# HanielUlises/GCN-GrabCut

Hardware: AMD Instinct MI355X
Metric: images/sec end-to-end mask (DUTS-shape batch) (higher is better)
Workload: dtype f32

## Files before the change

### gcn-grabcut_amd/csrc/ggc_ccl.h

```cpp
#pragma once
#include <hip/hip_runtime.h>
#include <cstdint>

namespace ggc {

__device__ __forceinline__ int ccl_find(const int32_t* parent, int i) {
    int p = __hip_atomic_load(&parent[i], __ATOMIC_RELAXED, __HIP_MEMORY_SCOPE_AGENT);
    while (p != i) { i = p; p = __hip_atomic_load(&parent[i], __ATOMIC_RELAXED, __HIP_MEMORY_SCOPE_AGENT); }
    return i;
}
__device__ __forceinline__ void ccl_union(int32_t* parent, int a, int b) {
    for (;;) {
        a = ccl_find(parent, a); b = ccl_find(parent, b);
        if (a == b) return;
        if (a < b) { const int t = a; a = b; b = t; }
        const int old = atomicMin(&parent[a], b);
        if (old == a) return;
        a = old;
    }
}

__host__ __device__ inline int ccl_run_start_lane(unsigned long long starts, int lane) {
    const unsigned long long below = starts & ((2ull << lane) - 1ull);
#if defined(__HIP_DEVICE_COMPILE__)
    return 63 - __clzll((long long)below);
#else
    return 63 - __builtin_clzll(below);
#endif
}
__host__ __device__ inline int ccl_run_length(unsigned long long starts, unsigned long long vmask, int lane) {
    const unsigned long long stop = (starts | ~vmask) >> lane >> 1;
#if defined(__HIP_DEVICE_COMPILE__)
    return stop ? __ffsll((long long)stop) : 64 - lane;
#else
    return stop ? __builtin_ffsll((long long)stop) : 64 - lane;
#endif
}

__device__ __forceinline__ int ccl_run_first(bool on, bool same_left, int p) {
    const int lane = threadIdx.x & 63;
    const unsigned long long starts = __ballot(on && (!same_left || lane == 0));
    return p - (lane - ccl_run_start_lane(starts, lane));
}

template <int CONN, class Joined>
__device__ __forceinline__ void ccl_merge_pixel(int32_t* par, int p, int x, bool has_up, int W, size_t flat, Joined joined) {
    static_assert(CONN == 4 || CONN == 8, "4 or 8 neighbours");
    const bool left = x > 0 && joined(p - 1);
    if (left && (flat & 63) == 0) ccl_union(par, p, p - 1);
    if (!has_up) return;
    if constexpr (CONN == 4) {
        if (joined(p - W) && !(left && joined(p - W - 1))) ccl_union(par, p, p - W);
    } else {
        const bool up = joined(p - W);
        const bool ul = x > 0 && joined(p - W - 1), ur = x + 1 < W && joined(p - W + 1);
        if (left) {
            if (ur && !up) ccl_union(par, p, p - W + 1);
        } else if (up) {
            ccl_union(par, p, p - W);
        } else {
            if (ul) ccl_union(par, p, p - W - 1);
            if (ur) ccl_union(par, p, p - W + 1);
        }
    }
}

__device__ __forceinline__ int ccl_compress(int32_t* par, int p) { const int r = ccl_find(par, p); par[p] = r; return r; }
__device__ __forceinline__ void ccl_count_runs(bool valid, bool same_left, unsigned long long vmask, int32_t* counts, size_t cell) {
    const int lane = threadIdx.x & 63;
    const unsigned long long starts = __ballot(valid && (!same_left || lane == 0));
    if (valid && ((starts >> lane) & 1ull)) atomicAdd(&counts[cell], ccl_run_length(starts, vmask, lane));
}

__host__ __device__ inline unsigned long long ccl_best_key(int area, int root) {
    return ((unsigned long long)(unsigned)area << 32) | (unsigned long long)(0xFFFFFFFFu - (unsigned)root);
}
__host__ __device__ inline int ccl_best_root(unsigned long long key) { return (int)(0xFFFFFFFFu - (unsigned)(key & 0xFFFFFFFFull)); }

}
```

### gcn-grabcut_amd/csrc/ggc_slic.hip

```cpp
#include "ggc_internal.h"
#include "ggc_ccl.h"
#include "ggc_math.h"
#include <cmath>
#include <vector>

namespace ggc {

__global__ void k_minmax_init(int B, uint32_t* mm) {
    const int i = blockIdx.x * blockDim.x + threadIdx.x;
    if (i < B) { mm[2 * i] = 0xFFFFFFFFu; mm[2 * i + 1] = 0u; }
}

__global__ void __launch_bounds__(256) k_minmax(size_t n, const float* __restrict__ img, uint32_t* mm) {
    const float* im = img + (size_t)blockIdx.y * n;
    float lo = INFINITY, hi = -INFINITY;
    for (size_t i = (size_t)blockIdx.x * blockDim.x + threadIdx.x; i < n; i += (size_t)gridDim.x * blockDim.x) {
        const float v = im[i];
        lo = fminf(lo, v); hi = fmaxf(hi, v);
    }
    for (int o = 32; o > 0; o >>= 1) { lo = fminf(lo, __shfl_xor(lo, o, 64)); hi = fmaxf(hi, __shfl_xor(hi, o, 64)); }
    __shared__ float s_lo[4], s_hi[4];
    if ((threadIdx.x & 63) == 0) { s_lo[threadIdx.x >> 6] = lo; s_hi[threadIdx.x >> 6] = hi; }
    __syncthreads();
    if (threadIdx.x == 0) {
// ... 83 lines not shown
__global__ void __launch_bounds__(256) k_gauss_v(int H, int W, const float* __restrict__ in, GaussW g, float* __restrict__ out) {
    const int col = blockIdx.x * 256 + threadIdx.x;
    if (col >= 3 * W) return;
    const size_t n = (size_t)H * W * 3;
    const float* im = in + (size_t)blockIdx.z * n + col;
    float* o = out + (size_t)blockIdx.z * n + col;
    const int y0 = blockIdx.y * GV_ROWS;
    double v[2 * R + 1];
#pragma unroll
    for (int j = 0; j < 2 * R; ++j) v[j + 1] = (double)im[(size_t)reflect_sym(y0 - R + j, H) * W * 3];
#pragma unroll 4
    for (int y = y0; y < min(y0 + GV_ROWS, H); ++y) {
#pragma unroll
        for (int j = 0; j < 2 * R; ++j) v[j] = v[j + 1];
        v[2 * R] = (double)im[(size_t)reflect_sym(y + R, H) * W * 3];
        double tmp = v[R] * g.w[R];
#pragma unroll
        for (int k = 0; k < R; ++k) tmp += (v[k] + v[2 * R - k]) * g.w[k];
        o[(size_t)y * W * 3] = (float)tmp;
    }
}

__global__ void __launch_bounds__(256) k_scale(size_t n, const float* __restrict__ in, float scale,
                                               float* __restrict__ out) {
    const size_t i = (size_t)blockIdx.x * blockDim.x + threadIdx.x;
    if (i < n) out[i] = in[i] * scale;
}

struct SlicGeom {
    int H, W, K;
    int ny, nx, start_y, start_x, step_y, step_x;
    int win_y, win_x;
    float sw;
};

__device__ __forceinline__ int4 slic_window(float cy, float cx, const SlicGeom& g) {
    if (cy != cy || cx != cx) return make_int4(0, 0, 0, 0);
    float fy0 = cy - (float)(2 * g.win_y); if (!(fy0 > 0.0f)) fy0 = 0.0f;
    float fy1 = cy + (float)(2 * g.win_y) + 1.0f; if (!(fy1 < (float)g.H)) fy1 = (float)g.H;
    float fx0 = cx - (float)(2 * g.win_x); if (!(fx0 > 0.0f)) fx0 = 0.0f;
    float fx1 = cx + (float)(2 * g.win_x) + 1.0f; if (!(fx1 < (float)g.W)) fx1 = (float)g.W;
    return make_int4((int)fy0, (int)fy1, (int)fx0, (int)fx1);
}

__global__ void k_init_centers(SlicGeom g, float* __restrict__ centers, int4* __restrict__ bounds) {
    const int k = blockIdx.x * blockDim.x + threadIdx.x;
    if (k >= g.K) return;
    const size_t o = (size_t)blockIdx.y * g.K + k;
    const float cy = (float)(g.start_y + (k / g.nx) * g.step_y);
    const float cx = (float)(g.start_x + (k % g.nx) * g.step_x);
    centers[o * 5 + 0] = cy; centers[o * 5 + 1] = cx;
    centers[o * 5 + 2] = 0.0f; centers[o * 5 + 3] = 0.0f; centers[o * 5 + 4] = 0.0f;
    bounds[o] = slic_window(cy, cx, g);
}

struct Cand { int k, y0, y1, x0, x1; float cy, cx, c0, c1, c2; };

constexpr int TILE_W = 32, TILE_H = 16;

typedef float v2f __attribute__((ext_vector_type(2)));

__global__ void __launch_bounds__(256) k_slic_assign(SlicGeom g, const float* __restrict__ image,
                                                     const float* __restrict__ centers,
                                                     const int4* __restrict__ bounds,
                                                     int32_t* __restrict__ labels, int32_t* __restrict__ stale) {
    __shared__ Cand cand[256];
    __shared__ int wcount[4];
    const int tid = threadIdx.x, lane = tid & 63, wave = tid >> 6;
    const int b = blockIdx.z;
    const int tx0 = blockIdx.x * TILE_W, ty0 = blockIdx.y * TILE_H;
    const int px = tx0 + (wave & 1) * 16 + (lane & 15), pya = ty0 + (wave >> 1) * 8 + (lane >> 4), pyb = pya + 4;
    const bool ina = px < g.W && pya < g.H, inb = px < g.W && pyb < g.H;
    const size_t P = (size_t)g.H * g.W;
    const size_t pa = (size_t)b * P + (size_t)pya * g.W + px, pb = pa + (size_t)4 * g.W;
    v2f i0 = 0.f, i1 = 0.f, i2 = 0.f;
    if (ina) { i0.x = image[3 * pa]; i1.x = image[3 * pa + 1]; i2.x = image[3 * pa + 2]; }
    if (inb) { i0.y = image[3 * pb]; i1.y = image[3 * pb + 1]; i2.y = image[3 * pb + 2]; }
    const v2f fy = {(float)pya, (float)pyb};
    const float fx = (float)px;
    float best_a = INFINITY, best_b = INFINITY;
    int lab_a = -1, lab_b = -1;
    const float* cen = centers + (size_t)b * g.K * 5;
    const int4* bnd = bounds + (size_t)b * g.K;
    for (int base = 0; base < g.K; base += 256) {
        const int k = base + tid;
        bool hit = false;
        int4 bd = make_int4(0, 0, 0, 0);
        if (k < g.K) {
            bd = bnd[k];
            hit = bd.x < ty0 + TILE_H && bd.y > ty0 && bd.z < tx0 + TILE_W && bd.w > tx0 && bd.y > bd.x && bd.w > bd.z;
        }
        const unsigned long long bal = __ballot(hit);
        const int pre = __popcll(bal & ((1ull << lane) - 1ull));
        if (lane == 0) wcount[wave] = __popcll(bal);
        __syncthreads();
        int off = 0, total = 0;
#pragma unroll
        for (int w = 0; w < 4; ++w) { if (w < wave) off += wcount[w]; total += wcount[w]; }
        if (hit) {
            Cand c;
            c.k = k; c.y0 = bd.x; c.y1 = bd.y; c.x0 = bd.z; c.x1 = bd.w;
            c.cy = cen[k * 5 + 0]; c.cx = cen[k * 5 + 1];
            c.c0 = cen[k * 5 + 2]; c.c1 = cen[k * 5 + 3]; c.c2 = cen[k * 5 + 4];
            cand[off + pre] = c;
        }
        __syncthreads();
        for (int i = 0; i < total; ++i) {
            const Cand& c = cand[i];
            const bool xin = (unsigned)(px - c.x0) < (unsigned)(c.x1 - c.x0);
            const unsigned hgt = (unsigned)(c.y1 - c.y0);
            const bool hit_a = xin && (unsigned)(pya - c.y0) < hgt, hit_b = xin && (unsigned)(pyb - c.y0) < hgt;
            if (!(hit_a || hit_b)) continue;
            const v2f ty = c.cy - fy;
            const float tx = c.cx - fx;
            v2f dd = (ty * ty + tx * tx) * g.sw;
            v2f t = i0 - c.c0;
            v2f dc = t * t;
            t = i1 - c.c1; dc += t * t;
            t = i2 - c.c2; dc += t * t;
            dd += dc;
            if (hit_a && best_a > dd.x) { best_a = dd.x; lab_a = c.k; }
            if (hit_b && best_b > dd.y) { best_b = dd.y; lab_b = c.k; }
        }
        __syncthreads();
    }
    bool none = false;
    if (ina) { if (lab_a >= 0) labels[pa] = lab_a; else none = true; }
    if (inb) { if (lab_b >= 0) labels[pb] = lab_b; else none = true; }
    if (none) atomicOr(&stale[b], 1);
}

constexpr int UPD_LANES = 8, UPD_GROUPS = 64 / UPD_LANES, UPD_CH = 8;
constexpr int UPD_CAP = 32;
constexpr int UPD_FOLD_UNROLL = 4;
static_assert(UPD_CAP >= 2 * UPD_LANES && UPD_CAP % UPD_FOLD_UNROLL == 0, "a fold per chunk, or fold reads past the list");

__device__ __forceinline__ void upd_wave_sync() {
    __builtin_amdgcn_fence(__ATOMIC_ACQ_REL, "wavefront");
    __builtin_amdgcn_wave_barrier();
}

__global__ void __launch_bounds__(256) k_slic_update(SlicGeom g, const float* __restrict__ image,
                                                     const int32_t* __restrict__ labels,
                                                     const int32_t* __restrict__ stale,
                                                     float* __restrict__ centers, int4* __restrict__ bounds) {
    __shared__ float upd_buf[4][UPD_CAP][UPD_GROUPS * 3];
    const int lane = threadIdx.x & 63, sub = lane / UPD_LANES, sl = lane % UPD_LANES;
    const int k = (blockIdx.x * 4 + (threadIdx.x >> 6)) * UPD_GROUPS + sub;
    const bool live = k < g.K;
    const int b = blockIdx.y;
    const size_t o = (size_t)b * g.K + (live ? k : 0);
    int4 bd = live ? bounds[o] : make_int4(0, 0, 0, 0);
    if (live && stale[b]) bd = make_int4(0, g.H, 0, g.W);
    const size_t P = (size_t)g.H * g.W;
    const int32_t* lb = labels + (size_t)b * P;
    const float* im = image + (size_t)b * P * 3;
    float s = 0.f;
    int cnt = 0, isy = 0, isx = 0;
    int nbuf = 0;
    float* const put = &upd_buf[threadIdx.x >> 6][0][sub * 3];
    const float* const get = put + min(sl, 2);
    auto fold = [&]() {
        upd_wave_sync();
        for (int i = 0; __any(i < nbuf); i += UPD_FOLD_UNROLL) {
            float v[UPD_FOLD_UNROLL];
#pragma unroll
            for (int u = 0; u < UPD_FOLD_UNROLL; ++u) v[u] = get[(i + u) * (UPD_GROUPS * 3)];
#pragma unroll
            for (int u = 0; u < UPD_FOLD_UNROLL; ++u) s += i + u < nbuf ? v[u] : 0.f;
        }
        nbuf = 0;
        upd_wave_sync();
    };
    const int rows = bd.y - bd.x, chunks = (bd.w - bd.z + UPD_LANES - 1) / UPD_LANES;
    int rows_max = rows, chunks_max = chunks;
#pragma unroll
    for (int off = UPD_LANES; off < 64; off <<= 1) {
        rows_max = max(rows_max, __shfl_xor(rows_max, off, 64));
        chunks_max = max(chunks_max, __shfl_xor(chunks_max, off, 64));
    }
    rows_max = __builtin_amdgcn_readfirstlane(rows_max);
    chunks_max = __builtin_amdgcn_readfirstlane(chunks_max);
    const int32_t* lane_p = lb + (size_t)bd.x * g.W + bd.z + sl;
    const int nvc = (bd.w - bd.z - sl + UPD_LANES - 1) / UPD_LANES;
    auto load_row = [&](int ry, int c0, int (&lab)[UPD_CH]) {
        const int32_t* rp = lane_p + (size_t)ry * g.W + c0 * UPD_LANES;
        const int nv = ry < rows ? nvc - c0 : 0;
#pragma unroll
        for (int c = 0; c < UPD_CH; ++c) lab[c] = c < nv ? rp[c * UPD_LANES] : -1;
    };
    const int nblk = (chunks_max + UPD_CH - 1) / UPD_CH, total = rows_max * nblk;
    int cur[UPD_CH], nxt[UPD_CH];
    if (total > 0) load_row(0, 0, cur);
    asm volatile("" :: "v"(cur[0]), "v"(cur[1]), "v"(cur[2]), "v"(cur[3]), "v"(cur[4]), "v"(cur[5]), "v"(cur[6]), "v"(cur[7]));
    int ry = 0, cb = 0;
    for (int t = 0; t < total; ++t) {
        int ry_n = ry, cb_n = cb + 1;
        if (cb_n == nblk) { cb_n = 0; ++ry_n; }
        load_row(ry_n, cb_n * UPD_CH, nxt);
        bool hit[UPD_CH], some = false;
#pragma unroll
        for (int c = 0; c < UPD_CH; ++c) { hit[c] = cur[c] == k && live; some |= hit[c]; }
        if (__any(some)) {
            const int y = bd.x + ry, x0 = bd.z + cb * UPD_CH * UPD_LANES + sl;
            const float* px = im + ((size_t)y * g.W + x0) * 3;
            float v0[UPD_CH], v1[UPD_CH], v2[UPD_CH];
#pragma unroll
            for (int c = 0; c < UPD_CH; ++c) {
                const float* q = hit[c] ? px + c * UPD_LANES * 3 : im;
                v0[c] = q[0]; v1[c] = q[1]; v2[c] = q[2];
            }
#pragma unroll
            for (int c = 0; c < UPD_CH; ++c) {
                const unsigned long long bal = __ballot(hit[c]);
                if (bal) {
                    if (__any(nbuf > UPD_CAP - UPD_LANES)) fold();
                    const unsigned int m = (unsigned int)(bal >> (sub * UPD_LANES)) & ((1u << UPD_LANES) - 1u);
                    const int n = __popc(m);
                    cnt += n; isy += n * y;
                    if (hit[c]) {
                        float* e = put + (nbuf + __popc(m & ((1u << sl) - 1u))) * (UPD_GROUPS * 3);
                        e[0] = v0[c]; e[1] = v1[c]; e[2] = v2[c];
                        isx += x0 + c * UPD_LANES;
                    }
                    nbuf += n;
                }
            }
        }
#pragma unroll
        for (int c = 0; c < UPD_CH; ++c) cur[c] = nxt[c];
        ry = ry_n; cb = cb_n;
    }
    fold();
    const float s0 = __shfl(s, lane - sl, 64), s1 = __shfl(s, lane - sl + 1, 64), s2 = __shfl(s, lane - sl + 2, 64);
#pragma unroll
    for (int off = 1; off < UPD_LANES; off <<= 1) isx += __shfl_xor(isx, off, 64);
    float sy = (float)isy, sx = (float)isx;
    if (live && (isy >= (1 << 24) || isx >= (1 << 24))) {
        sy = 0.f; sx = 0.f;
        for (int y = bd.x; y < bd.y; ++y)
            for (int x = bd.z; x < bd.w; ++x)
                if (lb[(size_t)y * g.W + x] == k) { sy += (float)y; sx += (float)x; }
    }
    if (!live || sl != 0) return;
    const float n = (float)cnt;
    const float cy = sy / n, cx = sx / n;
    centers[o * 5 + 0] = cy; centers[o * 5 + 1] = cx;
    centers[o * 5 + 2] = s0 / n; centers[o * 5 + 3] = s1 / n; centers[o * 5 + 4] = s2 / n;
    bounds[o] = slic_window(cy, cx, g);
}

__global__ void __launch_bounds__(64) k_connectivity_seq(int H, int W, const int32_t* __restrict__ labels,
                                                         int min_size, int max_size,
                                                         int32_t* __restrict__ queue,
                                                         int32_t* __restrict__ out, int32_t* __restrict__ n_nodes) {
    if (threadIdx.x != 0) return;
    const int b = blockIdx.x;
    const size_t P = (size_t)H * W;
    const int32_t* lb = labels + (size_t)b * P;
    int32_t* o = out + (size_t)b * P;
    int32_t* q = queue + (size_t)b * (size_t)(max_size > 0 ? max_size : 1);
    int cur = 0;
    for (int y = 0; y < H; ++y)
        for (int x = 0; x < W; ++x) {
            const int p0 = y * W + x;
            if (o[p0] >= 0) continue;
            int adjacent = 0;
            const int label = lb[p0];
            o[p0] = cur;
            int size = 1, visited = 0;
            q[0] = p0;
            while (visited < size && size < max_size) {
                const int pc = q[visited];
                const int yc = pc / W, xc = pc - yc * W;
#pragma unroll
                for (int i = 0; i < 4; ++i) {
                    const int xx = xc + (i == 0 ? 1 : i == 1 ? -1 : 0);
                    const int yy = yc + (i == 2 ? 1 : i == 3 ? -1 : 0);
                    if (xx < 0 || xx >= W || yy < 0 || yy >= H) continue;
                    const int pp = yy * W + xx;
                    const int op = o[pp];
                    if (op == -1 && lb[pp] == label) {
                        o[pp] = cur;
                        q[size] = pp;
                        size += 1;
                        if (size >= max_size) break;
                    } else if (op >= 0 && op != cur) {
                        adjacent = op;
                    }
                }
                visited += 1;
            }
            if (size < min_size) {
                for (int i = 0; i < size; ++i) o[q[i]] = adjacent;
            } else {
                cur += 1;
            }
        }
    n_nodes[b] = cur > 0 ? cur : 1;
}

struct CnDims { int B, H, W, P, min_size, max_size; };

__global__ void __launch_bounds__(256) k_cn_reset(CnDims d, const int32_t* __restrict__ raw, const uint8_t* __restrict__ pending,
                                                  int32_t* __restrict__ parent, int32_t* __restrict__ csize) {
    const size_t i = (size_t)blockIdx.x * blockDim.x + threadIdx.x;
    const bool valid = i < (size_t)d.B * d.P && pending[i];
    bool same_left = false;
    int p = 0;
    if (valid) {
        p = (int)(i % d.P);
        same_left = (p % d.W) > 0 && pending[i - 1] && raw[i - 1] == raw[i];
    }
    const int first = ccl_run_first(valid, same_left, p);
    if (!valid) return;
    parent[i] = first;
    csize[i] = 0;
}

__global__ void __launch_bounds__(256) k_cn_merge(CnDims d, const int32_t* __restrict__ raw, const uint8_t* __restrict__ pending,
                                                  int32_t* __restrict__ parent) {
    const int x = blockIdx.x * 64 + (threadIdx.x & 63), y = blockIdx.y * 4 + (threadIdx.x >> 6);
    if (x >= d.W || y >= d.H) return;
    const size_t base = (size_t)blockIdx.z * d.P;
    const int p = y * d.W + x;
    if (!pending[base + p]) return;
    const int l = raw[base + p];
    ccl_merge_pixel<4>(parent + base, p, x, y > 0, d.W, base + p, [=](int q) { return pending[base + q] && raw[base + q] == l; });
}

__global__ void __launch_bounds__(256) k_cn_size(CnDims d, const int32_t* __restrict__ raw, const uint8_t* __restrict__ pending,
                                                 int32_t* __restrict__ parent, int32_t* __restrict__ csize) {
    const size_t i = (size_t)blockIdx.x * blockDim.x + threadIdx.x;
    const bool valid = i < (size_t)d.B * d.P && pending[i];
    bool same_left = false;
    size_t base = 0;
    int r = 0;
    if (valid) {
        base = (i / d.P) * d.P;
        const int p = (int)(i - base);
        same_left = (p % d.W) > 0 && pending[i - 1] && raw[i - 1] == raw[i];
        r = ccl_compress(parent + base, p);
    }
    ccl_count_runs(valid, same_left, __ballot(valid), csize, base + r);
}

__global__ void __launch_bounds__(256) k_cn_settle(CnDims d, uint8_t* __restrict__ pending, const int32_t* __restrict__ parent,
                                                   const int32_t* __restrict__ csize, int32_t* __restrict__ n_big) {
    const size_t i = (size_t)blockIdx.x * blockDim.x + threadIdx.x;
    if (i >= (size_t)d.B * d.P || !pending[i]) return;
    const size_t base = (i / d.P) * d.P;
    const int p = (int)(i - base), r = parent[i];
    if (csize[base + r] < d.max_size) pending[i] = 0;
    else if (p == r) atomicAdd(n_big, 1);
}

__global__ void __launch_bounds__(64) k_cn_carve(CnDims d, int tag, uint8_t* __restrict__ pending, const int32_t* __restrict__ parent,
                                                 int32_t* __restrict__ csize, int32_t* __restrict__ mark,
                                                 int32_t* __restrict__ queue, int32_t* __restrict__ qtop) {
    const size_t i = (size_t)blockIdx.x * blockDim.x + threadIdx.x;
    if (i >= (size_t)d.B * d.P) return;
    const int b = (int)(i / d.P);
    const size_t base = (size_t)b * d.P;
    const int r = (int)(i - base);
    if (!pending[i] || parent[i] != r || csize[i] < d.max_size) return;
    int32_t* q = queue + base + atomicAdd(&qtop[b], d.max_size);
    int size = 1, visited = 0;
    q[0] = r; mark[base + r] = tag;
    while (visited < size && size < d.max_size) {
        const int pc = q[visited];
        const int yc = pc / d.W, xc = pc - yc * d.W;
#pragma unroll
        for (int k = 0; k < 4; ++k) {
            const int xx = xc + (k == 0 ? 1 : k == 1 ? -1 : 0), yy = yc + (k == 2 ? 1 : k == 3 ? -1 : 0);
            if (xx < 0 || xx >= d.W || yy < 0 || yy >= d.H) continue;
            const int pp = yy * d.W + xx;
            if (pending[base + pp] && parent[base + pp] == r && mark[base + pp] != tag) {
                mark[base + pp] = tag;
                q[size++] = pp;
                if (size >= d.max_size) break;
            }
        }
        visited += 1;
    }
    for (int k = 0; k < size; ++k) pending[base + q[k]] = 0;
    csize[i] = size;
}

__global__ void __launch_bounds__(256) k_cn_kept(CnDims d, const int32_t* __restrict__ parent, const int32_t* __restrict__ csize,
                                                 int32_t* __restrict__ rank) {
    const size_t i = (size_t)blockIdx.x * blockDim.x + threadIdx.x;
    if (i >= (size_t)d.B * d.P) return;
    rank[i] = (parent[i] == (int)(i % d.P) && csize[i] >= d.min_size) ? 1 : 0;
}

__global__ void __launch_bounds__(1024) k_cn_scan(CnDims d, int32_t* __restrict__ rank, int32_t* __restrict__ n_nodes) {
    __shared__ int32_t wsum[16];
    __shared__ int32_t s_carry;
    const int b = blockIdx.x, tid = threadIdx.x, lane = tid & 63, wave = tid >> 6;
    int32_t* a = rank + (size_t)b * d.P;
    if (tid == 0) s_carry = 0;
    __syncthreads();
    for (int base = 0; base < d.P; base += 4096) {
        const int i0 = base + tid * 4;
        int32_t c[4], s = 0;
#pragma unroll
        for (int j = 0; j < 4; ++j) { c[j] = i0 + j < d.P ? a[i0 + j] : 0; s += c[j]; }
        int32_t incl = s;
        for (int o = 1; o < 64; o <<= 1) { const int32_t v = __shfl_up(incl, o, 64); if (lane >= o) incl += v; }
        if (lane == 63) wsum[wave] = incl;
        __syncthreads();
        int32_t run = s_carry + (incl - s), total = 0;
#pragma unroll
        for (int w = 0; w < 16; ++w) { if (w < wave) run += wsum[w]; total += wsum[w]; }
#pragma unroll
        for (int j = 0; j < 4; ++j) { if (i0 + j < d.P) a[i0 + j] = run; run += c[j]; }
        __syncthreads();
        if (tid == 0) s_carry += total;
        __syncthreads();
    }
    if (tid == 0) n_nodes[b] = s_carry > 0 ? s_carry : 1;
}

__global__ void __launch_bounds__(64) k_cn_small(CnDims d, int tag, const int32_t* __restrict__ parent,
                                                 const int32_t* __restrict__ csize, int32_t* __restrict__ mark,
                                                 int32_t* __restrict__ queue, int32_t* __restrict__ qtop,
                                                 int32_t* __restrict__ tgt) {
    const size_t i = (size_t)blockIdx.x * blockDim.x + threadIdx.x;
    if (i >= (size_t)d.B * d.P) return;
    const int b = (int)(i / d.P);
    const size_t base = (size_t)b * d.P;
    const int r = (int)(i - base);
    if (parent[i] != r || csize[i] >= d.min_size) return;
    const int n = csize[i];
    int32_t* q = queue + base + atomicAdd(&qtop[b], n);
    int size = 1, visited = 0, last = -1;
    q[0] = r; mark[base + r] = tag;
    while (visited < size) {
        const int pc = q[visited];
        const int yc = pc / d.W, xc = pc - yc * d.W;
#pragma unroll
        for (int k = 0; k < 4; ++k) {
            const int xx = xc + (k == 0 ? 1 : k == 1 ? -1 : 0), yy = yc + (k == 2 ? 1 : k == 3 ? -1 : 0);
            if (xx < 0 || xx >= d.W || yy < 0 || yy >= d.H) continue;
            const int pp = yy * d.W + xx;
            const int rp = parent[base + pp];
            if (rp == r) { if (mark[base + pp] != tag && size < n) { mark[base + pp] = tag; q[size++] = pp; } }
            else if (rp < r) last = rp;
        }
        visited += 1;
    }
    tgt[i] = last;
}

__global__ void __launch_bounds__(256) k_cn_write(CnDims d, const int32_t* __restrict__ parent, const int32_t* __restrict__ csize,
                                                  const int32_t* __restrict__ rank, const int32_t* __restrict__ tgt,
                                                  int32_t* __restrict__ out) {
    const size_t i = (size_t)blockIdx.x * blockDim.x + threadIdx.x;
    if (i >= (size_t)d.B * d.P) return;
    const size_t base = (i / d.P) * d.P;
    int r = parent[i];
    int lab = 0;
    for (;;) {
        if (csize[base + r] >= d.min_size) { lab = rank[base + r]; break; }
        const int t = tgt[base + r];
        if (t < 0) { lab = 0; break; }
        r = t;
    }
    out[i] = lab;
}


static double np_pairwise_sum(const double* a, int n) {
    if (n < 8) { double s = 0.0; for (int i = 0; i < n; ++i) s += a[i]; return s; }
    double r[8];
    for (int j = 0; j < 8; ++j) r[j] = a[j];
    int i;
    for (i = 8; i < n - (n % 8); i += 8) for (int j = 0; j < 8; ++j) r[j] += a[i + j];
    double res = ((r[0] + r[1]) + (r[2] + r[3])) + ((r[4] + r[5]) + (r[6] + r[7]));
    for (; i < n; ++i) res += a[i];
    return res;
}

struct Grid { int step_y, step_x, start_y, start_x, ny, nx, K; };
static Grid regular_grid(int H, int W, int n_points) {
    Grid g{};
    const double dims[3] = {1.0, (double)(H <= W ? H : W), (double)(H <= W ? W : H)};
    const double space = 1.0 * H * W;
    if (space <= (double)n_points) { g = {1, 1, 0, 0, H, W, H * W}; return g; }
    double st[3];
    for (int i = 0; i < 3; ++i) st[i] = std::pow(space / n_points, 1.0 / 3.0);
    if (dims[0] < st[0] || dims[1] < st[1] || dims[2] < st[2]) {
        for (int dim = 0; dim < 3; ++dim) {
            st[dim] = dims[dim];
            double sp = 1.0;
            for (int j = dim + 1; j < 3; ++j) sp *= dims[j];
            for (int j = dim + 1; j < 3; ++j) st[j] = std::pow(sp / n_points, 1.0 / (3 - dim - 1));
            if (dims[0] >= st[0] && dims[1] >= st[1] && dims[2] >= st[2]) break;
        }
    }
    int starts[3], steps[3];
    for (int i = 0; i < 3; ++i) { starts[i] = (int)std::floor(st[i] / 2.0); steps[i] = (int)std::rint(st[i]); }
    const int iy = (H <= W) ? 1 : 2, ix = (H <= W) ? 2 : 1;
    g.step_y = steps[iy]; g.start_y = starts[iy];
    g.step_x = steps[ix]; g.start_x = starts[ix];
    g.ny = std::max(0, (H - g.start_y + g.step_y - 1) / g.step_y);
    g.nx = std::max(0, (W - g.start_x + g.step_x - 1) / g.step_x);
    g.K = g.ny * g.nx;
    return g;
}

}

using namespace ggc;

static int enforce_connectivity(ggc_ctx* ctx, hipStream_t st, int B, int H, int W, const int32_t* raw, int min_size,
                                int max_size, int32_t* segments, int32_t* n_nodes) {
    const size_t P = (size_t)H * W;
    if (knobs().slic_seq_connectivity) {
        int32_t* queue = scratch_t<int32_t>(ctx, S_SLIC_AUX3, (size_t)B * (size_t)std::max(max_size, 1));
        if (!queue) return GGC_E_OOM;
        GGC_HIP(ctx, hipMemsetAsync(segments, 0xFF, sizeof(int32_t) * (size_t)B * P, st));
        ProfScope prof(ctx, st, "slic_connectivity");
        hipLaunchKernelGGL(k_connectivity_seq, dim3(B), dim3(64), 0, st, H, W, raw, min_size, max_size, queue, segments,
                           n_nodes);
        GGC_LAUNCH_CHECK(ctx);
        return GGC_OK;
    }
    {
        ProfScope prof(ctx, st, "slic_connectivity");
        const size_t BP = (size_t)B * P;
        const CnDims cd{B, H, W, (int)P, min_size, std::max(max_size, 1)};
        int32_t* work = scratch_t<int32_t>(ctx, S_SLIC_AUX3, BP * 6 + (size_t)B * (size_t)cd.max_size + 2 * (size_t)B + 16);
        uint8_t* pending = scratch_t<uint8_t>(ctx, S_SLIC_AUX4, BP);
        if (!work || !pending) return GGC_E_OOM;
        int32_t *parent = work, *csize = work + BP, *rank = work + 2 * BP, *tgt = work + 3 * BP, *mark = work + 4 * BP;
        int32_t* queue = work + 5 * BP;
        int32_t* qtop = work + 6 * BP + (size_t)B * cd.max_size;
        int32_t* n_big = qtop + B;
        GGC_HIP(ctx, hipMemsetAsync(pending, 1, BP, st));
        GGC_HIP(ctx, hipMemsetAsync(mark, 0, sizeof(int32_t) * BP, st));
        const dim3 g1(cdiv(BP, 256)), g2(cdiv(W, 64), cdiv(H, 4), B), g64(cdiv(BP, 64));
        for (int round = 0; round < 4096; ++round) {
            GGC_HIP(ctx, hipMemsetAsync(qtop, 0, sizeof(int32_t) * (B + 1), st));
            hipLaunchKernelGGL(k_cn_reset, g1, dim3(256), 0, st, cd, raw, pending, parent, csize);
            hipLaunchKernelGGL(k_cn_merge, g2, dim3(256), 0, st, cd, raw, pending, parent);
            hipLaunchKernelGGL(k_cn_size, g1, dim3(256), 0, st, cd, raw, pending, parent, csize);
            hipLaunchKernelGGL(k_cn_settle, g1, dim3(256), 0, st, cd, pending, parent, csize, n_big);
            GGC_LAUNCH_CHECK(ctx);
            int32_t h_big = 0;
            GGC_HIP(ctx, hipMemcpyAsync(&h_big, n_big, sizeof(int32_t), hipMemcpyDeviceToHost, st));
            GGC_HIP(ctx, hipStreamSynchronize(st));
            if (h_big == 0) break;
            hipLaunchKernelGGL(k_cn_carve, g64, dim3(64), 0, st, cd, round + 1, pending, parent, csize, mark, queue, qtop);
            GGC_LAUNCH_CHECK(ctx);
        }
        hipLaunchKernelGGL(k_cn_kept, g1, dim3(256), 0, st, cd, parent, csize, rank);
        hipLaunchKernelGGL(k_cn_scan, dim3(B), dim3(1024), 0, st, cd, rank, n_nodes);
        GGC_HIP(ctx, hipMemsetAsync(qtop, 0, sizeof(int32_t) * (B + 1), st));
        hipLaunchKernelGGL(k_cn_small, g64, dim3(64), 0, st, cd, 0x7FFFFFFF, parent, csize, mark, queue, qtop, tgt);
        hipLaunchKernelGGL(k_cn_write, g1, dim3(256), 0, st, cd, parent, csize, rank, tgt, segments);
        GGC_LAUNCH_CHECK(ctx);
    }
    return GGC_OK;
}

extern "C" int ggc_slic(ggc_ctx* ctx, ggc_stream stream, int B, int H, int W, const float* image,
                        int n_segments, float compactness, float sigma, int rescale_input,
                        int32_t* segments, int32_t* n_nodes) {
    if (!ctx) return GGC_E_INVALID_ARG;
    GGC_REQUIRE(ctx, B >= 1 && H >= 1 && W >= 1 && B <= 65535, GGC_E_SHAPE, "bad shape B=%d H=%d W=%d", B, H, W);
    GGC_REQUIRE(ctx, image && segments && n_nodes, GGC_E_INVALID_ARG, "null pointer");
    GGC_REQUIRE(ctx, n_segments >= 1 && compactness > 0.0f && sigma >= 0.0f, GGC_E_INVALID_ARG,
                "bad SLIC parameters n_segments=%d compactness=%g sigma=%g", n_segments, compactness, sigma);
    GGC_REQUIRE(ctx, (size_t)H * W < (1u << 30), GGC_E_SHAPE, "image too large");
    GGC_HIP(ctx, hipSetDevice(ctx->device));
    hipStream_t st = reinterpret_cast<hipStream_t>(stream);
    const size_t P = (size_t)H * W;

    const Grid seed = regular_grid(H, W, n_segments);
    GGC_REQUIRE(ctx, seed.K >= 1, GGC_E_SHAPE, "no SLIC seeds for %dx%d with n_segments=%d", H, W, n_segments);
    const Grid win = regular_grid(H, W, seed.K);
    SlicGeom g{};
    g.H = H; g.W = W; g.K = seed.K;
    g.ny = seed.ny; g.nx = seed.nx; g.start_y = seed.start_y; g.start_x = seed.start_x;
    g.step_y = seed.step_y; g.step_x = seed.step_x;
    g.win_y = win.step_y; g.win_x = win.step_x;
    const float step = (float)std::max(std::max(seed.step_y, seed.step_x), 1);
    g.sw = (float)(1.0 / (double)(step * step));

    float* img_a = scratch_t<float>(ctx, S_SLIC_IMG, (size_t)B * P * 3);
    float* img_b = scratch_t<float>(ctx, S_SLIC_TMP, (size_t)B * P * 3);
    uint32_t* mm = scratch_t<uint32_t>(ctx, S_SLIC_MINMAX, (size_t)B * 2);
    float* centers = scratch_t<float>(ctx, S_SLIC_CENTERS, (size_t)B * g.K * 5);
    int4* bounds = scratch_t<int4>(ctx, S_SLIC_AUX, (size_t)B * g.K);
    int32_t* raw = scratch_t<int32_t>(ctx, S_SLIC_LABELS, (size_t)B * P);
    int32_t* stale = scratch_t<int32_t>(ctx, S_SLIC_AUX2, (size_t)B * 10);
    if (!img_a || !img_b || !mm || !centers || !bounds || !raw || !stale) return GGC_E_OOM;

    hipLaunchKernelGGL(k_minmax_init, dim3(cdiv(B, 256)), dim3(256), 0, st, B, mm);
    hipLaunchKernelGGL(k_minmax, dim3(std::min(cdiv(P * 3, 256 * 8), 48), B), dim3(256), 0, st, P * 3, image, mm);
    hipLaunchKernelGGL(k_lab2, dim3(cdiv(P, 256), B), dim3(256), 0, st, P, image, mm, rescale_input, img_a);
    GGC_LAUNCH_CHECK(ctx);
    const float ratio = (float)(1.0 / (double)compactness);
    const float* km_img = nullptr;
    if (sigma > 0.0f) {
        GaussW gw{};
        gw.r = (int)(4.0 * (double)sigma + 0.5);
        GGC_REQUIRE(ctx, gw.r <= MAX_RADIUS, GGC_E_UNSUPPORTED, "sigma=%g needs radius %d > %d", sigma, gw.r, MAX_RADIUS);
        ggc_gaussian_taps((double)sigma, gw.r, gw.w);
        const double sum = np_pairwise_sum(gw.w, 2 * gw.r + 1);
        for (int i = 0; i < 2 * gw.r + 1; ++i) gw.w[i] = gw.w[i] / sum;
        GGC_REQUIRE(ctx, H <= 65535, GGC_E_SHAPE, "H=%d exceeds the launch grid", H);
        const dim3 grid(cdiv((size_t)W * 3, 256), H, B);
        if (gw.r == 4) {
            hipLaunchKernelGGL((k_gauss_v<4>), dim3(cdiv((size_t)W * 3, 256), cdiv(H, GV_ROWS), B), dim3(256), 0, st, H, W, img_a, gw, img_b);
            hipLaunchKernelGGL((k_gauss<1, 4>), grid, dim3(256), 0, st, H, W, img_b, gw, ratio, 1, img_a);
        } else {
            hipLaunchKernelGGL((k_gauss<0, 0>), grid, dim3(256), 0, st, H, W, img_a, gw, 1.0f, 0, img_b);
            hipLaunchKernelGGL((k_gauss<1, 0>), grid, dim3(256), 0, st, H, W, img_b, gw, ratio, 1, img_a);
        }
        km_img = img_a;
    } else {
        hipLaunchKernelGGL(k_scale, dim3(cdiv((size_t)B * P * 3, 256)), dim3(256), 0, st, (size_t)B * P * 3, img_a,
                           ratio, img_b);
        km_img = img_b;
    }
    GGC_LAUNCH_CHECK(ctx);
    hipLaunchKernelGGL(k_init_centers, dim3(cdiv(g.K, 256), B), dim3(256), 0, st, g, centers, bounds);
    GGC_HIP(ctx, hipMemsetAsync(raw, 0, sizeof(int32_t) * (size_t)B * P, st));
    GGC_HIP(ctx, hipMemsetAsync(stale, 0, sizeof(int32_t) * (size_t)B * 10, st));
    for (int it = 0; it < 10; ++it) {
        {
            ProfScope prof(ctx, st, "slic_assign");
            hipLaunchKernelGGL(k_slic_assign, dim3(cdiv(W, TILE_W), cdiv(H, TILE_H), B), dim3(256), 0, st, g, km_img,
                               centers, bounds, raw, stale + (size_t)it * B);
        }
        if (it < 9) {
            ProfScope prof(ctx, st, "slic_update");
            hipLaunchKernelGGL(k_slic_update, dim3(cdiv(g.K, 4 * UPD_GROUPS), B), dim3(256), 0, st, g, km_img, raw,
                               stale + (size_t)it * B, centers, bounds);
        }
        GGC_LAUNCH_CHECK(ctx);
    }
    const double seg_size = (double)P / (double)g.K;
    const int min_size = (int)(0.5 * seg_size), max_size = (int)(3.0 * seg_size);
    return enforce_connectivity(ctx, st, B, H, W, raw, min_size, max_size, segments, n_nodes);
}

namespace ggc {

__global__ void __launch_bounds__(256) k_minmax_u8(size_t n, const uint8_t* __restrict__ img, int32_t* __restrict__ mm) {
    const uint8_t* im = img + (size_t)blockIdx.y * n;
    int lo = 255, hi = 0;
    for (size_t i = (size_t)blockIdx.x * blockDim.x + threadIdx.x; i < n; i += (size_t)gridDim.x * blockDim.x) {
        const int v = im[i];
        lo = min(lo, v); hi = max(hi, v);
    }
    for (int o = 32; o > 0; o >>= 1) { lo = min(lo, __shfl_xor(lo, o, 64)); hi = max(hi, __shfl_xor(hi, o, 64)); }
    if ((threadIdx.x & 63) == 0) { atomicMin(&mm[2 * blockIdx.y], lo); atomicMax(&mm[2 * blockIdx.y + 1], hi); }
}
__global__ void k_minmax_u8_init(int B, int32_t* mm) {
    const int i = blockIdx.x * blockDim.x + threadIdx.x;
    if (i < B) { mm[2 * i] = 255; mm[2 * i + 1] = 0; }
}

__global__ void __launch_bounds__(256) k_rgb_lab64(size_t P, const uint8_t* __restrict__ bgr, const int32_t* __restrict__ mm,
                                                   GaussW g, int smooth, double* __restrict__ out) {
    const size_t p = (size_t)blockIdx.x * blockDim.x + threadIdx.x;
    if (p >= P) return;
    const size_t base = ((size_t)blockIdx.y * P + p) * 3;
    const double mn = (double)mm[2 * blockIdx.y], mx = (double)mm[2 * blockIdx.y + 1];
    const double range = mx - mn;
    double lin[3];
#pragma unroll
    for (int c = 0; c < 3; ++c) {
        double v = (double)bgr[base + 2 - c];
        v = v - mn; if (mx != mn) v = v / range;
        lin[c] = v > 0.04045 ? det_pow24((v + 0.055) / 1.055) : v / 12.92;
    }
    const double X = (lin[0] * 0.412453 + lin[1] * 0.357580) + lin[2] * 0.180423;
    const double Y = (lin[0] * 0.212671 + lin[1] * 0.715160) + lin[2] * 0.072169;
    const double Z = (lin[0] * 0.019334 + lin[1] * 0.119193) + lin[2] * 0.950227;
    const double t[3] = {X / 0.95047, Y / 1.0, Z / 1.08883};
    double f[3];
#pragma unroll
    for (int c = 0; c < 3; ++c) f[c] = t[c] > 0.008856 ? det_cbrt(t[c]) : 7.787 * t[c] + 16.0 / 116.0;
    double lab[3] = {116.0 * f[1] - 16.0, 500.0 * (f[0] - f[1]), 200.0 * (f[1] - f[2])};
    if (smooth) {
#pragma unroll
        for (int c = 0; c < 3; ++c) {
            double tmp = lab[c] * g.w[g.r];
            for (int jj = -g.r; jj < 0; ++jj) tmp += (lab[c] + lab[c]) * g.w[jj + g.r];
            lab[c] = tmp;
        }
    }
    out[base + 0] = lab[0]; out[base + 1] = lab[1]; out[base + 2] = lab[2];
}

template <int AXIS>
__global__ void __launch_bounds__(256) k_gauss64(int H, int W, const double* __restrict__ in, GaussW g, double scale,
                                                 int apply_scale, double* __restrict__ out) {
    const int col = blockIdx.x * 256 + threadIdx.x;
    if (col >= 3 * W) return;
    const int y = blockIdx.y;
    const size_t n = (size_t)H * W * 3;
    const double* im = in + (size_t)blockIdx.z * n;
    const int x = col / 3, c = col - 3 * x;
    const int l = AXIS == 0 ? y : x;
    const int len = AXIS == 0 ? H : W;
    auto at = [&](int idx) -> double {
        const int j = reflect_sym(idx, len);
        return AXIS == 0 ? im[((size_t)j * W + x) * 3 + c] : im[((size_t)y * W + j) * 3 + c];
    };
    double tmp = at(l) * g.w[g.r];
    for (int jj = -g.r; jj < 0; ++jj) tmp += (at(l + jj) + at(l - jj)) * g.w[jj + g.r];
    if (apply_scale) tmp = tmp * scale;
    out[(size_t)blockIdx.z * n + (size_t)y * W * 3 + col] = tmp;
}
__global__ void __launch_bounds__(256) k_scale64(size_t n, const double* __restrict__ in, double scale, double* __restrict__ out) {
    const size_t i = (size_t)blockIdx.x * blockDim.x + threadIdx.x;
    if (i < n) out[i] = in[i] * scale;
}

__device__ __forceinline__ int4 slic_window64(double cy, double cx, const SlicGeom& g) {
    if (cy != cy || cx != cx) return make_int4(0, 0, 0, 0);
    double fy0 = cy - (double)(2 * g.win_y); if (!(fy0 > 0.0)) fy0 = 0.0;
    double fy1 = cy + (double)(2 * g.win_y) + 1.0; if (!(fy1 < (double)g.H)) fy1 = (double)g.H;
    double fx0 = cx - (double)(2 * g.win_x); if (!(fx0 > 0.0)) fx0 = 0.0;
    double fx1 = cx + (double)(2 * g.win_x) + 1.0; if (!(fx1 < (double)g.W)) fx1 = (double)g.W;
    return make_int4((int)fy0, (int)fy1, (int)fx0, (int)fx1);
}
__global__ void k_init_centers64(SlicGeom g, double* __restrict__ centers, int4* __restrict__ bounds) {
    const int k = blockIdx.x * blockDim.x + threadIdx.x;
    if (k >= g.K) return;
    const size_t o = (size_t)blockIdx.y * g.K + k;
    const double cy = (double)(g.start_y + (k / g.nx) * g.step_y), cx = (double)(g.start_x + (k % g.nx) * g.step_x);
    centers[o * 5 + 0] = cy; centers[o * 5 + 1] = cx;
    centers[o * 5 + 2] = 0.0; centers[o * 5 + 3] = 0.0; centers[o * 5 + 4] = 0.0;
    bounds[o] = slic_window64(cy, cx, g);
}

struct Cand64 { int k, y0, y1, x0, x1; double cy, cx, c0, c1, c2; };

__global__ void __launch_bounds__(256) k_slic_assign64(SlicGeom g, double sw, const double* __restrict__ image,
                                                       const double* __restrict__ centers, const int4* __restrict__ bounds,
                                                       int32_t* __restrict__ labels, int32_t* __restrict__ stale) {
    __shared__ Cand64 cand[256];
    __shared__ int wcount[4];
    const int tid = threadIdx.x, lane = tid & 63, wave = tid >> 6;
    const int b = blockIdx.z;
    const int tx0 = blockIdx.x * 32, ty0 = blockIdx.y * 8;
    const int px = tx0 + (tid & 31), py = ty0 + (tid >> 5);
    const bool in = px < g.W && py < g.H;
    const size_t P = (size_t)g.H * g.W;
    const size_t p = (size_t)b * P + (size_t)py * g.W + px;
    double i0 = 0.0, i1 = 0.0, i2 = 0.0;
    if (in) { i0 = image[3 * p]; i1 = image[3 * p + 1]; i2 = image[3 * p + 2]; }
    double best = INFINITY;
    int lab = -1;
    const double* cen = centers + (size_t)b * g.K * 5;
    const int4* bnd = bounds + (size_t)b * g.K;
    for (int base = 0; base < g.K; base += 256) {
        const int k = base + tid;
        bool hit = false;
        int4 bd = make_int4(0, 0, 0, 0);
        if (k < g.K) {
            bd = bnd[k];
            hit = bd.x < ty0 + 8 && bd.y > ty0 && bd.z < tx0 + 32 && bd.w > tx0 && bd.y > bd.x && bd.w > bd.z;
        }
        const unsigned long long bal = __ballot(hit);
        const int pre = __popcll(bal & ((1ull << lane) - 1ull));
        if (lane == 0) wcount[wave] = __popcll(bal);
        __syncthreads();
        int off = 0, total = 0;
#pragma unroll
        for (int w = 0; w < 4; ++w) { if (w < wave) off += wcount[w]; total += wcount[w]; }
        if (hit) {
            Cand64 c;
            c.k = k; c.y0 = bd.x; c.y1 = bd.y; c.x0 = bd.z; c.x1 = bd.w;
            c.cy = cen[k * 5 + 0]; c.cx = cen[k * 5 + 1]; c.c0 = cen[k * 5 + 2]; c.c1 = cen[k * 5 + 3]; c.c2 = cen[k * 5 + 4];
            cand[off + pre] = c;
        }
        __syncthreads();
        for (int i = 0; i < total; ++i) {
            const Cand64& c = cand[i];
            if (!((unsigned)(px - c.x0) < (unsigned)(c.x1 - c.x0) && (unsigned)(py - c.y0) < (unsigned)(c.y1 - c.y0))) continue;
            const double ty = c.cy - (double)py, tx = c.cx - (double)px;
            double dd = (ty * ty + tx * tx) * sw;
            double t = i0 - c.c0, dc = t * t;
            t = i1 - c.c1; dc += t * t;
            t = i2 - c.c2; dc += t * t;
            dd += dc;
            if (best > dd) { best = dd; lab = c.k; }
        }
        __syncthreads();
    }
    if (in) { if (lab >= 0) labels[p] = lab; else atomicOr(&stale[b], 1); }
}

__global__ void __launch_bounds__(256) k_slic_update64(SlicGeom g, const double* __restrict__ image, const int32_t* __restrict__ labels,
                                                       const int32_t* __restrict__ stale, double* __restrict__ centers,
                                                       int4* __restrict__ bounds) {
    const int lane = threadIdx.x & 63, sub = lane / UPD_LANES, sl = lane % UPD_LANES;
    const int k = (blockIdx.x * 4 + (threadIdx.x >> 6)) * UPD_GROUPS + sub;
    const bool live = k < g.K;
    const int b = blockIdx.y;
    const size_t o = (size_t)b * g.K + (live ? k : 0);
    int4 bd = live ? bounds[o] : make_int4(0, 0, 0, 0);
    if (live && stale[b]) bd = make_int4(0, g.H, 0, g.W);
    const size_t P = (size_t)g.H * g.W;
    const int32_t* lb = labels + (size_t)b * P;
    const double* im = image + (size_t)b * P * 3;
    double s0 = 0.0, s1 = 0.0, s2 = 0.0;
    long long cnt = 0, isy = 0, isx = 0;
    const int rows = bd.y - bd.x, cols = bd.w - bd.z;
    int rows_max = rows, cols_max = cols;
#pragma unroll
    for (int off = UPD_LANES; off < 64; off <<= 1) {
        rows_max = max(rows_max, __shfl_xor(rows_max, off, 64));
        cols_max = max(cols_max, __shfl_xor(cols_max, off, 64));
    }
    for (int ry = 0; ry < rows_max; ++ry) {
        const int y = bd.x + ry;
        for (int c0 = 0; c0 < cols_max; c0 += UPD_LANES) {
            const int x = bd.z + c0 + sl;
            const bool hit = live && ry < rows && x < bd.w && lb[(size_t)y * g.W + x] == k;
            const unsigned long long bal = __ballot(hit);
            if (!bal) continue;
            unsigned int m = (unsigned int)(bal >> (sub * UPD_LANES)) & ((1u << UPD_LANES) - 1u);
            double v0 = 0.0, v1 = 0.0, v2 = 0.0;
            if (hit) { const double* px = im + ((size_t)y * g.W + x) * 3; v0 = px[0]; v1 = px[1]; v2 = px[2]; isx += x; }
            const int n = __popc(m);
            cnt += n; isy += (long long)n * y;
            while (__any(m != 0u)) {
                const int src = sub * UPD_LANES + (m ? __ffs((int)m) - 1 : 0);
                const double t0 = __shfl(v0, src, 64), t1 = __shfl(v1, src, 64), t2 = __shfl(v2, src, 64);
                if (m) { s0 += t0; s1 += t1; s2 += t2; }
                m &= m - 1u;
            }
        }
    }
#pragma unroll
    for (int off = 1; off < UPD_LANES; off <<= 1) isx += __shfl_xor(isx, off, 64);
    if (!live || sl != 0) return;
    const double n = (double)cnt;
    const double cy = (double)isy / n, cx = (double)isx / n;
    centers[o * 5 + 0] = cy; centers[o * 5 + 1] = cx;
    centers[o * 5 + 2] = s0 / n; centers[o * 5 + 3] = s1 / n; centers[o * 5 + 4] = s2 / n;
    bounds[o] = slic_window64(cy, cx, g);
}

}

extern "C" int ggc_slic_rgb(ggc_ctx* ctx, ggc_stream stream, int B, int H, int W, const uint8_t* bgr, int n_segments,
                            double compactness, double sigma, int32_t* segments, int32_t* n_nodes) {
    if (!ctx) return GGC_E_INVALID_ARG;
    GGC_REQUIRE(ctx, B >= 1 && H >= 1 && W >= 1 && B <= 65535 && H <= 65535, GGC_E_SHAPE, "bad shape B=%d H=%d W=%d", B, H, W);
    GGC_REQUIRE(ctx, bgr && segments && n_nodes, GGC_E_INVALID_ARG, "null pointer");
    GGC_REQUIRE(ctx, n_segments >= 1 && compactness > 0.0 && sigma >= 0.0, GGC_E_INVALID_ARG,
// ... 76 lines not shown
```

Measured before the change: 3820.

## Tile SLIC connectivity labelling in LDS with border merge and tile-local size counting

```diff
diff --git a/gcn-grabcut_amd/csrc/ggc_ccl.h b/gcn-grabcut_amd/csrc/ggc_ccl.h
--- a/gcn-grabcut_amd/csrc/ggc_ccl.h
+++ b/gcn-grabcut_amd/csrc/ggc_ccl.h
@@ -72,6 +72,69 @@
     if (valid && ((starts >> lane) & 1ull)) atomicAdd(&counts[cell], ccl_run_length(starts, vmask, lane));
 }
 
+constexpr int CCL_TILE_W = 64;
+
+__device__ __forceinline__ int ccl_lds_find(const int32_t* f, int i) {
+    int p = __hip_atomic_load(&f[i], __ATOMIC_RELAXED, __HIP_MEMORY_SCOPE_WORKGROUP);
+    while ((unsigned)p < (unsigned)i) { i = p; p = __hip_atomic_load(&f[i], __ATOMIC_RELAXED, __HIP_MEMORY_SCOPE_WORKGROUP); }
+    return i;
+}
+__device__ __forceinline__ void ccl_lds_union(int32_t* f, int a, int b) {
+    for (;;) {
+        a = ccl_lds_find(f, a); b = ccl_lds_find(f, b);
+        if (a == b) return;
+        if (a < b) { const int t = a; a = b; b = t; }
+        const int old = atomicMin(&f[a], b);
+        if (old == a) return;
+        a = old;
+    }
+}
+
+__device__ __forceinline__ void ccl_tile_init_row(int32_t* f, int32_t* key, int ly, bool on, int32_t k) {
+    const int lane = threadIdx.x & 63, l = ly * CCL_TILE_W + lane;
+    const int32_t kl = __shfl_up(k, 1, 64);
+    const bool onl = __shfl_up((int)on, 1, 64) != 0;
+    const int first = ccl_run_first(on, lane > 0 && onl && kl == k, l);
+    f[l] = on ? first : -1;
+    key[l] = k;
+}
+__device__ __forceinline__ void ccl_tile_merge_pixel(int32_t* f, const int32_t* key, int l) {
+    const int32_t k = key[l];
+    auto joined = [&](int q) { return __hip_atomic_load(&f[q], __ATOMIC_RELAXED, __HIP_MEMORY_SCOPE_WORKGROUP) >= 0 && key[q] == k; };
+    const bool left = (l & (CCL_TILE_W - 1)) > 0 && joined(l - 1);
+    if (joined(l - CCL_TILE_W) && !(left && joined(l - CCL_TILE_W - 1))) ccl_lds_union(f, l, l - CCL_TILE_W);
+}
+__device__ __forceinline__ int ccl_tile_global(int l, int W, int tx0, int ty0) {
+    return (ty0 + l / CCL_TILE_W) * W + tx0 + (l & (CCL_TILE_W - 1));
+}
+template <int TH>
+__device__ __forceinline__ int ccl_tile_local(int v, int W, int tx0, int ty0) {
+    const int vy = v / W, ly = vy - ty0, lx = v - vy * W - tx0;
+    return ((unsigned)ly < (unsigned)TH && (unsigned)lx < (unsigned)CCL_TILE_W) ? ly * CCL_TILE_W + lx : -1;
+}
+
+template <int TH, class Joined>
+__device__ __forceinline__ void ccl_tile_border_pixel(int32_t* par, int p, int x, int y, int W, Joined joined) {
+    const bool col = x > 0 && x % CCL_TILE_W == 0, row = y > 0 && y % TH == 0;
+    if (!col && !row) return;
+    const bool left = x > 0 && joined(p - 1);
+    if (col && left && !(y % TH != 0 && joined(p - W) && joined(p - W - 1))) ccl_union(par, p, p - 1);
+    if (row && joined(p - W) && !(left && joined(p - W - 1))) ccl_union(par, p, p - W);
+}
+
+__device__ __forceinline__ int ccl_tile_exit(const int32_t* link, int l) {
+    int e = link[l];
+    while ((unsigned)e < (unsigned)l) { l = e; e = link[l]; }
+    return l;
+}
+__device__ __forceinline__ void ccl_tile_count_runs(int e, int32_t* cnt) {
+    const int lane = threadIdx.x & 63;
+    const int el = __shfl_up(e, 1, 64);
+    const bool on = e >= 0;
+    const unsigned long long vmask = __ballot(on), starts = __ballot(on && (lane == 0 || el != e));
+    if (on && ((starts >> lane) & 1ull)) atomicAdd(&cnt[e], ccl_run_length(starts, vmask, lane));
+}
+
 __host__ __device__ inline unsigned long long ccl_best_key(int area, int root) {
     return ((unsigned long long)(unsigned)area << 32) | (unsigned long long)(0xFFFFFFFFu - (unsigned)root);
 }
diff --git a/gcn-grabcut_amd/csrc/ggc_slic.hip b/gcn-grabcut_amd/csrc/ggc_slic.hip
--- a/gcn-grabcut_amd/csrc/ggc_slic.hip
+++ b/gcn-grabcut_amd/csrc/ggc_slic.hip
@@ -409,57 +409,111 @@
 
 struct CnDims { int B, H, W, P, min_size, max_size; };
 
-__global__ void __launch_bounds__(256) k_cn_reset(CnDims d, const int32_t* __restrict__ raw, const uint8_t* __restrict__ pending,
-                                                  int32_t* __restrict__ parent, int32_t* __restrict__ csize) {
-    const size_t i = (size_t)blockIdx.x * blockDim.x + threadIdx.x;
-    const bool valid = i < (size_t)d.B * d.P && pending[i];
-    bool same_left = false;
-    int p = 0;
-    if (valid) {
-        p = (int)(i % d.P);
-        same_left = (p % d.W) > 0 && pending[i - 1] && raw[i - 1] == raw[i];
-    }
-    const int first = ccl_run_first(valid, same_left, p);
-    if (!valid) return;
-    parent[i] = first;
-    csize[i] = 0;
-}
-
-__global__ void __launch_bounds__(256) k_cn_merge(CnDims d, const int32_t* __restrict__ raw, const uint8_t* __restrict__ pending,
-                                                  int32_t* __restrict__ parent) {
-    const int x = blockIdx.x * 64 + (threadIdx.x & 63), y = blockIdx.y * 4 + (threadIdx.x >> 6);
+constexpr int CN_TH = 16;
+constexpr int CN_TILE = CCL_TILE_W * CN_TH;
+static_assert(CN_TH % 4 == 0, "four waves share a tile's rows");
+
+template <bool FIRST>
+__global__ void __launch_bounds__(256) k_cn_tile(CnDims d, const int32_t* __restrict__ raw, uint8_t* __restrict__ pending,
+                                                 int32_t* __restrict__ parent, int32_t* __restrict__ csize) {
+    __shared__ int32_t forest[CN_TILE], key[CN_TILE];
+    const int lane = threadIdx.x & 63, wave = threadIdx.x >> 6;
+    const int tx0 = blockIdx.x * CCL_TILE_W, ty0 = blockIdx.y * CN_TH, x = tx0 + lane;
+    const size_t base = (size_t)blockIdx.z * d.P;
+#pragma unroll
+    for (int j = 0; j < CN_TH / 4; ++j) {
+        const int ly = j * 4 + wave, y = ty0 + ly;
+        const size_t i = base + (size_t)y * d.W + x;
+        bool on = x < d.W && y < d.H;
+        int32_t k = 0;
+        if (on) {
+            if (FIRST) pending[i] = 1; else on = pending[i] != 0;
+            k = raw[i];
+        }
+        ccl_tile_init_row(forest, key, ly, on, k);
+    }
+    __syncthreads();
+#pragma unroll
+    for (int j = 0; j < CN_TH / 4; ++j) {
+        const int l = (j * 4 + wave) * CCL_TILE_W + lane;
+        if (l >= CCL_TILE_W && forest[l] >= 0) ccl_tile_merge_pixel(forest, key, l);
+    }
+    __syncthreads();
+#pragma unroll
+    for (int j = 0; j < CN_TH / 4; ++j) {
+        const int ly = j * 4 + wave, l = ly * CCL_TILE_W + lane;
+        if (forest[l] < 0) continue;
+        const size_t i = base + (size_t)(ty0 + ly) * d.W + x;
+        parent[i] = ccl_tile_global(ccl_lds_find(forest, l), d.W, tx0, ty0);
+        csize[i] = 0;
+    }
+}
+
+__global__ void __launch_bounds__(128) k_cn_border(CnDims d, const int32_t* __restrict__ raw, const uint8_t* __restrict__ pending,
+                                                   int32_t* __restrict__ parent) {
+    const int t = threadIdx.x;
+    if (t >= CCL_TILE_W + CN_TH || t == CCL_TILE_W) return;
+    const int x = blockIdx.x * CCL_TILE_W + (t < CCL_TILE_W ? t : 0), y = blockIdx.y * CN_TH + (t < CCL_TILE_W ? 0 : t - CCL_TILE_W);
     if (x >= d.W || y >= d.H) return;
     const size_t base = (size_t)blockIdx.z * d.P;
     const int p = y * d.W + x;
     if (!pending[base + p]) return;
     const int l = raw[base + p];
-    ccl_merge_pixel<4>(parent + base, p, x, y > 0, d.W, base + p, [=](int q) { return pending[base + q] && raw[base + q] == l; });
-}
-
-__global__ void __launch_bounds__(256) k_cn_size(CnDims d, const int32_t* __restrict__ raw, const uint8_t* __restrict__ pending,
-                                                 int32_t* __restrict__ parent, int32_t* __restrict__ csize) {
+    ccl_tile_border_pixel<CN_TH>(parent + base, p, x, y, d.W, [=](int q) { return pending[base + q] && raw[base + q] == l; });
+}
+
+__global__ void __launch_bounds__(256) k_cn_size(CnDims d, const uint8_t* __restrict__ pending, int32_t* __restrict__ parent,
+                                                 int32_t* __restrict__ csize) {
+    __shared__ int32_t link[CN_TILE], groot[CN_TILE], cnt[CN_TILE];
+    const int lane = threadIdx.x & 63, wave = threadIdx.x >> 6;
+    const int tx0 = blockIdx.x * CCL_TILE_W, ty0 = blockIdx.y * CN_TH, x = tx0 + lane;
+    const size_t base = (size_t)blockIdx.z * d.P;
+#pragma unroll
+    for (int j = 0; j < CN_TH / 4; ++j) {
+        const int ly = j * 4 + wave, y = ty0 + ly, l = ly * CCL_TILE_W + lane;
+        const int p = y * d.W + x;
+        int lk = -1;
+        if (x < d.W && y < d.H && pending[base + p]) {
+            const int v = parent[base + p];
+            lk = v != p ? ccl_tile_local<CN_TH>(v, d.W, tx0, ty0) : -1;
+            if (lk < 0) { lk = l; groot[l] = v != p ? ccl_find(parent + base, v) : p; cnt[l] = 0; }
+        }
+        link[l] = lk;
+    }
+    __syncthreads();
+#pragma unroll
+    for (int j = 0; j < CN_TH / 4; ++j) {
+        const int ly = j * 4 + wave, l = ly * CCL_TILE_W + lane;
+        int e = -1;
+        if (link[l] >= 0) {
+            e = ccl_tile_exit(link, l);
+            parent[base + (size_t)(ty0 + ly) * d.W + x] = groot[e];
+        }
+        ccl_tile_count_runs(e, cnt);
+    }
+    __syncthreads();
+#pragma unroll
+    for (int j = 0; j < CN_TH / 4; ++j) {
+        const int l = (j * 4 + wave) * CCL_TILE_W + lane;
+        if (link[l] == l) atomicAdd(&csize[base + groot[l]], cnt[l]);
+    }
+}
+
+__global__ void __launch_bounds__(256) k_cn_settle(CnDims d, uint8_t* __restrict__ pending, const int32_t* __restrict__ parent,
+                                                   const int32_t* __restrict__ csize, int32_t* __restrict__ n_big,
+                                                   int32_t* __restrict__ rank) {
     const size_t i = (size_t)blockIdx.x * blockDim.x + threadIdx.x;
-    const bool valid = i < (size_t)d.B * d.P && pending[i];
-    bool same_left = false;
-    size_t base = 0;
-    int r = 0;
-    if (valid) {
-        base = (i / d.P) * d.P;
-        const int p = (int)(i - base);
-        same_left = (p % d.W) > 0 && pending[i - 1] && raw[i - 1] == raw[i];
-        r = ccl_compress(parent + base, p);
-    }
-    ccl_count_runs(valid, same_left, __ballot(valid), csize, base + r);
-}
-
-__global__ void __launch_bounds__(256) k_cn_settle(CnDims d, uint8_t* __restrict__ pending, const int32_t* __restrict__ parent,
-                                                   const int32_t* __restrict__ csize, int32_t* __restrict__ n_big) {
-    const size_t i = (size_t)blockIdx.x * blockDim.x + threadIdx.x;
-    if (i >= (size_t)d.B * d.P || !pending[i]) return;
+    if (i >= (size_t)d.B * d.P) return;
     const size_t base = (i / d.P) * d.P;
     const int p = (int)(i - base), r = parent[i];
-    if (csize[base + r] < d.max_size) pending[i] = 0;
-    else if (p == r) atomicAdd(n_big, 1);
+    int n = 0;
+    if (p == r) n = csize[i];
+    if (pending[i]) {
+        if (p != r) n = csize[base + r];
+        if (n < d.max_size) pending[i] = 0;
+        else if (p == r) atomicAdd(n_big, 1);
+    }
+    rank[i] = (p == r && n >= d.min_size) ? 1 : 0;
 }
 
 __global__ void __launch_bounds__(64) k_cn_carve(CnDims d, int tag, uint8_t* __restrict__ pending, const int32_t* __restrict__ parent,
@@ -492,13 +546,6 @@
     }
     for (int k = 0; k < size; ++k) pending[base + q[k]] = 0;
     csize[i] = size;
-}
-
-__global__ void __launch_bounds__(256) k_cn_kept(CnDims d, const int32_t* __restrict__ parent, const int32_t* __restrict__ csize,
-                                                 int32_t* __restrict__ rank) {
-    const size_t i = (size_t)blockIdx.x * blockDim.x + threadIdx.x;
-    if (i >= (size_t)d.B * d.P) return;
-    rank[i] = (parent[i] == (int)(i % d.P) && csize[i] >= d.min_size) ? 1 : 0;
 }
 
 __global__ void __launch_bounds__(1024) k_cn_scan(CnDims d, int32_t* __restrict__ rank, int32_t* __restrict__ n_nodes) {
@@ -645,15 +692,15 @@
         int32_t* queue = work + 5 * BP;
         int32_t* qtop = work + 6 * BP + (size_t)B * cd.max_size;
         int32_t* n_big = qtop + B;
-        GGC_HIP(ctx, hipMemsetAsync(pending, 1, BP, st));
         GGC_HIP(ctx, hipMemsetAsync(mark, 0, sizeof(int32_t) * BP, st));
-        const dim3 g1(cdiv(BP, 256)), g2(cdiv(W, 64), cdiv(H, 4), B), g64(cdiv(BP, 64));
+        const dim3 g1(cdiv(BP, 256)), gt(cdiv(W, CCL_TILE_W), cdiv(H, CN_TH), B), g64(cdiv(BP, 64));
         for (int round = 0; round < 4096; ++round) {
             GGC_HIP(ctx, hipMemsetAsync(qtop, 0, sizeof(int32_t) * (B + 1), st));
-            hipLaunchKernelGGL(k_cn_reset, g1, dim3(256), 0, st, cd, raw, pending, parent, csize);
-            hipLaunchKernelGGL(k_cn_merge, g2, dim3(256), 0, st, cd, raw, pending, parent);
-            hipLaunchKernelGGL(k_cn_size, g1, dim3(256), 0, st, cd, raw, pending, parent, csize);
-            hipLaunchKernelGGL(k_cn_settle, g1, dim3(256), 0, st, cd, pending, parent, csize, n_big);
+            if (round == 0) hipLaunchKernelGGL(k_cn_tile<true>, gt, dim3(256), 0, st, cd, raw, pending, parent, csize);
+            else hipLaunchKernelGGL(k_cn_tile<false>, gt, dim3(256), 0, st, cd, raw, pending, parent, csize);
+            hipLaunchKernelGGL(k_cn_border, gt, dim3(128), 0, st, cd, raw, pending, parent);
+            hipLaunchKernelGGL(k_cn_size, gt, dim3(256), 0, st, cd, pending, parent, csize);
+            hipLaunchKernelGGL(k_cn_settle, g1, dim3(256), 0, st, cd, pending, parent, csize, n_big, rank);
             GGC_LAUNCH_CHECK(ctx);
             int32_t h_big = 0;
             GGC_HIP(ctx, hipMemcpyAsync(&h_big, n_big, sizeof(int32_t), hipMemcpyDeviceToHost, st));
@@ -662,7 +709,6 @@
             hipLaunchKernelGGL(k_cn_carve, g64, dim3(64), 0, st, cd, round + 1, pending, parent, csize, mark, queue, qtop);
             GGC_LAUNCH_CHECK(ctx);
         }
-        hipLaunchKernelGGL(k_cn_kept, g1, dim3(256), 0, st, cd, parent, csize, rank);
         hipLaunchKernelGGL(k_cn_scan, dim3(B), dim3(1024), 0, st, cd, rank, n_nodes);
         GGC_HIP(ctx, hipMemsetAsync(qtop, 0, sizeof(int32_t) * (B + 1), st));
         hipLaunchKernelGGL(k_cn_small, g64, dim3(64), 0, st, cd, 0x7FFFFFFF, parent, csize, mark, queue, qtop, tgt);
```

After: 3857 (median of 6 runs). No clear change (+1.0%).
